# dpfried/action-segmentation

Measured on AMD Instinct MI355X. Metric: frames/sec semi-Markov decode, CrossTask T~10k K~20 L=1024, 1/2/4/8 GPUs, higher is better.
Workload: dtype f64

## Files before the change

action-segmentation_amd/_lib.py:

```python
import ctypes
import os

HERE = os.path.dirname(os.path.abspath(__file__))
LIB_PATH = os.environ.get("SMM_LIB_PATH") or os.path.join(HERE, "libsmmdp.so")

SYMBOLS = [
    "smm_strerror", "smm_last_hip_error", "smm_version", "smm_device_count", "smm_workspace_bytes",
    "smm_error_word_offset", "smm_dp_timing_enable", "smm_dp_timing_read", "smm_dp_timing_read_tagged", "smm_band_frame_ns", "smm_time_split_plan",
    "smm_env_reload", "smm_release_cached_plans", "smm_cached_plan_bytes", "smm_plan_feedback_info", "smm_plan_feedback_plan",
    "smm_emission_f64", "smm_emission_bwd_f64", "smm_viterbi_f64", "smm_viterbi_f32", "smm_decode_f32", "smm_logz_f64", "smm_logz_bwd_f64",
    "smm_sample_f64", "smm_entropy_f64", "smm_segment_posteriors_f64", "smm_kl_f64", "smm_kbest_workspace_bytes", "smm_kbest_f64",
    "smm_mbr_workspace_bytes", "smm_mbr_f64",
    "smm_align_workspace_bytes", "smm_align_f64", "smm_align_opt_workspace_bytes", "smm_align_opt_f64",
    "smm_align_graph_workspace_bytes", "smm_align_graph_f64",
    "smm_align_logz_workspace_bytes", "smm_align_logz_f64", "smm_align_logz_bwd_f64",
    "smm_align_opt_logz_workspace_bytes", "smm_align_opt_logz_f64", "smm_align_opt_logz_bwd_f64",
    "smm_align_graph_logz_workspace_bytes", "smm_align_graph_logz_f64", "smm_align_graph_logz_bwd_f64",
    "smm_align_graph_sample_f64", "smm_align_graph_entropy_f64", "smm_align_graph_kl_f64",
    "smm_align_graph_segment_posteriors_f64",
    "smm_entropy_bwd_scratch_bytes", "smm_entropy_bwd_f64", "smm_kl_bwd_f64",
    "smm_expected_reward_bwd_scratch_bytes", "smm_expected_reward_f64", "smm_expected_reward_bwd_f64",
    "smm_align_graph_entropy_bwd_scratch_bytes", "smm_align_graph_entropy_bwd_f64", "smm_align_graph_kl_bwd_f64",
    "smm_factor_tables_f64", "smm_factor_tables_bwd_f64",
    "smm_dense_workspace_bytes", "smm_dense_dp_f32", "smm_dense_marginals_f32",
    "smm_eval_workspace_bytes", "smm_eval_confusion_i64", "smm_eval_videos_i64",
    "smm_fit_workspace_bytes", "smm_fit_error_word_offset", "smm_fit_stats_f64",
]


class SmmShape(ctypes.Structure):
    _fields_ = [("b", ctypes.c_int32), ("d", ctypes.c_int32), ("n_groups", ctypes.c_int32),
                ("c_max", ctypes.c_int32), ("k_rows", ctypes.c_int32), ("t_max", ctypes.c_int32),
                ("flags", ctypes.c_int32), ("total_frames", ctypes.c_int64)]


class SmmPlanFeedbackInfo(ctypes.Structure):
    _fields_ = [("n_replans", ctypes.c_int32), ("n1_before", ctypes.c_int32), ("n1_after", ctypes.c_int32),
                ("n_videos", ctypes.c_int32), ("end_before_us", ctypes.c_double), ("end_after_us", ctypes.c_double),
                ("stamps", ctypes.POINTER(ctypes.c_uint64)), ("order", ctypes.POINTER(ctypes.c_int32))]


class SmmTablesShape(ctypes.Structure):
    _fields_ = [("n_classes", ctypes.c_int32), ("d", ctypes.c_int32), ("n_groups", ctypes.c_int32),
                ("c_max", ctypes.c_int32), ("k_rows", ctypes.c_int32), ("allow_self_transitions", ctypes.c_int32)]


SHAPE_NO_EOS = 1
SHAPE_LOGZ_BOTH = 2
SHAPE_NO_TIME_SPLIT = 4
KL_BWD_CROSS_ENTROPY = 0
KL_BWD_KL = 1
MAX_TRANSCRIPT = 256
ALIGN_LOGZ_TILE = 768

# ... 146 lines not shown
    lib.smm_band_frame_ns.restype = ctypes.c_double
    lib.smm_band_frame_ns.argtypes = [ctypes.c_int]
    lib.smm_time_split_plan.restype = ctypes.c_int
    lib.smm_time_split_plan.argtypes = [ctypes.POINTER(SmmShape)] + [ctypes.c_void_p] * 4 + [ctypes.c_int] + [ctypes.c_void_p] * 4 + [ctypes.c_int]
    lib.smm_env_reload.restype = None
    lib.smm_env_reload.argtypes = []
    lib.smm_release_cached_plans.restype = ctypes.c_size_t
    lib.smm_release_cached_plans.argtypes = []
    lib.smm_cached_plan_bytes.restype = ctypes.c_size_t
    lib.smm_cached_plan_bytes.argtypes = []
    lib.smm_plan_feedback_info.restype = ctypes.c_int
    lib.smm_plan_feedback_info.argtypes = [ctypes.POINTER(SmmPlanFeedbackInfo)]
    lib.smm_plan_feedback_plan.restype = ctypes.c_int
    lib.smm_plan_feedback_plan.argtypes = [ctypes.c_int, ctypes.c_int, ctypes.c_double] + [ctypes.c_void_p] * 3 + [ctypes.c_int, ctypes.c_int] \
        + [ctypes.c_void_p] * 4
    _lib = lib
    return lib


def reload_env():
    if _lib is not None:
        _lib.smm_env_reload()


def check(status):
    if status != 0:
        lib = load()
        msg = lib.smm_strerror(status).decode()
        if status == -4:
            msg += " (hipError %d)" % lib.smm_last_hip_error()
# ... 24 lines not shown
```

action-segmentation_amd/csrc/smm_api.hip:

```cpp
#include <algorithm>
#include <atomic>
#include <functional>
#include <cstdio>
#include <cstdlib>
#include <cstring>
#include <numeric>
#include <vector>
#include <unordered_map>
#include <mutex>
#include <utility>
#include <string>

#include "../../include/smmdp.h"
#include "smm_device.h"
#include "smm_launch.h"
#include "smm_plan_feedback.h"

static thread_local int g_last_hip = 0;

namespace {
struct SmmEnv {
    int spec = 1;
    int no_split = 0;
    double split_min_us = 100.0, split_ns = 0.0;
    int split_margin = 400;
    int plan_cache = 1;
    int small_wg = 1;
    int plan_feedback = 1;
    int chunk = 1;
    int chunk_p = 0;
    int chunk_lmin = 0;
    int chunk_wc = 512;
    int no_bt_window = 0;
    int fit_grid = 0;
    int verbose = 0;
#ifdef SMM_DEV
    int debug_flags = 0;
    int split_debug = 0;
    int upload_memcpy = 0;
    int emission_v2 = 0;
#endif
    std::string key;
};
std::atomic<const SmmEnv *> g_env{nullptr};
std::once_flag g_env_once;

void env_read()
{
    SmmEnv e;
    struct Item { const char *name; int *i; double *d; };
    const Item items[] = {
        {"SMM_SPEC", &e.spec, nullptr}, {"SMM_NO_SPLIT", &e.no_split, nullptr}, {"SMM_SPLIT_MIN_US", nullptr, &e.split_min_us},
        {"SMM_SPLIT_NS", nullptr, &e.split_ns}, {"SMM_SPLIT_MARGIN", &e.split_margin, nullptr},
        {"SMM_PLAN_CACHE", &e.plan_cache, nullptr}, {"SMM_SMALL_WG", &e.small_wg, nullptr}, {"SMM_PLAN_FEEDBACK", &e.plan_feedback, nullptr}, {"SMM_CHUNK", &e.chunk, nullptr}, {"SMM_CHUNK_P", &e.chunk_p, nullptr},
        {"SMM_CHUNK_WC", &e.chunk_wc, nullptr}, {"SMM_CHUNK_LMIN", &e.chunk_lmin, nullptr}, {"SMM_NO_BT_WINDOW", &e.no_bt_window, nullptr},
        {"SMM_FIT_GRID", &e.fit_grid, nullptr}, {"SMM_VERBOSE", &e.verbose, nullptr},
#ifdef SMM_DEV
        {"SMM_DEBUG_FLAGS", &e.debug_flags, nullptr}, {"SMM_SPLIT_DEBUG", &e.split_debug, nullptr},
        {"SMM_UPLOAD_MEMCPY", &e.upload_memcpy, nullptr}, {"SMM_EMISSION_V2", &e.emission_v2, nullptr},
#endif
    };
    for (const Item &it : items) {
        const char *v = std::getenv(it.name);
        if (!v) continue;
        if (it.i) *it.i = (*v == 0) ? 1 : std::atoi(v);
        if (it.d) *it.d = std::atof(v);
        e.key += it.name; e.key += '='; e.key += v; e.key += ';';
    }
// ... 238 lines not shown
struct Staged {
    SmmVideo *videos;
    int32_t *order;
    int32_t *n_states;
    int32_t *err;
    double *hist;
    double *elp;
    double *tabs;
    double *band;
    bool band_mode;
    int32_t *em_cum;
    std::vector<int32_t> em_cum_host;
    int em_tpw, em_blocks;
    int kp_max, c_need;
    int n_split;
    SmmVideo *uvideos;
    int32_t *uorder, *porder;
    SmmChunkVideo *cvs;
    int32_t *redo;
    double *anchors;
    int n_cv, n_units, u_part1;
    int small_first, small_count;
    uint64_t *stamps = nullptr;
    hipEvent_t done = nullptr;
    void *fb_entry = nullptr;
    std::vector<int32_t> order_host, frames_host;
};

static bool band_mode(int kp_max, int c_need);

// ... 22 lines not shown
    const SmmEnv &ev = env();
    if (b < 24 || ev.no_split) return 0;
    const int n_cu = device_cus();
    if (n_cu <= 0) return 0;
    const double em_us = (double)total_frames * (4.0 * d + 8.0 * c_max) / 4.0e6;
    if (em_us < ev.split_min_us) return 0;
    int tmax = 0;
    for (int i = 0; i < b; ++i) tmax = std::max(tmax, hv[i].T);
    const double split_ns = ev.split_ns > 0.0 ? ev.split_ns : 1.75 * smm_band_frame_ns(std::min(c_max, (int)SMM_MAX_STATES));
    const int thr = tmax - (int)(em_us * 1000.0 / split_ns) - ev.split_margin;
    int n1 = 0;
    for (int i = 0; i < b; ++i) n1 += hv[i].T >= thr;
    if (thr <= 0 || n1 < 1 || n1 > b / 3 || n1 > n_cu / 2 || b - n1 < 16 || b > 2 * n_cu) return 0;
    std::stable_partition(order, order + b, [&](int32_t v) { return hv[v].T >= thr; });
    return n1;
}

namespace {
struct PlanFeedback {
    uint64_t *stamps = nullptr;
    hipEvent_t done = nullptr;
    bool pending = false;
    bool have = false;
    bool busy = false;
    int evals_left = 5, n_replans = 0;
    int b = 0, n1_first = 0;
    double em_us = 0.0, end_before_us = 0.0, end_after_us = 0.0;
    std::vector<uint64_t> snap, used;
    std::vector<int32_t> order, frames;
};
// ... 273 lines not shown
{
    std::lock_guard<std::mutex> lock(g_plans.mu);
    size_t n = g_plans.pinned_bytes;
    for (int d = 0; d < 64; ++d)
        for (auto &ps : g_plans.slabs[d].all) n += ps.second;
    return n;
}

namespace {
struct FeedbackInfo {
    uint64_t generation = 0;
    smm_plan_feedback_info_t info{};
};
thread_local FeedbackInfo g_fb_info;

void feedback_info_set(const PlanFeedback *fb, int n1_now)
{
    g_fb_info.generation = g_plans.generation;
    smm_plan_feedback_info_t &o = g_fb_info.info;
    o.n_replans = fb->n_replans;
    o.n1_before = fb->n1_first;
    o.n1_after = n1_now;
    o.n_videos = fb->b;
    o.end_before_us = fb->end_before_us;
    o.end_after_us = fb->end_after_us;
    o.stamps = fb->used.empty() ? nullptr : fb->used.data();
    o.order = fb->order.data();
}

void feedback_evaluate(const Staged &st, hipStream_t stream)
{
    PlanEntry *e = static_cast<PlanEntry *>(st.fb_entry);
    if (!e || !e->fb) return;
    PlanFeedback *fb = e->fb;
    std::vector<uint64_t> snap;
    std::vector<int32_t> order;
    int n1 = 0;
    {
        std::lock_guard<std::mutex> lock(g_plans.mu);
        if (!fb->have || fb->busy || fb->evals_left <= 0) { feedback_info_set(fb, e->st.n_split); return; }
        fb->busy = true;
        snap = fb->snap;
        order = fb->order;
        n1 = e->st.n_split;
    }
    const SmmEnv &ev = env();
    const int b = fb->b, n_cu = device_cus();
    std::vector<double> dur(b);
    for (int i = 0; i < b; ++i) dur[i] = (double)(snap[2 * i + 1] - snap[2 * i]) * 0.01;
    const bool force = ev.plan_feedback >= 2;
    double em_us = fb->em_us;
    {
        uint64_t s1 = ~0ull, s2 = ~0ull;
        double f1 = 0.0, f_all = 0.0;
        for (int i = 0; i < b; ++i) {
            const int v = order[i];
            (i < n1 ? s1 : s2) = std::min(i < n1 ? s1 : s2, snap[2 * (size_t)v]);
            f_all += fb->frames[v];
            if (i < n1) f1 += fb->frames[v];
        }
        if (s2 > s1 && f_all > f1) em_us = std::min(2.0 * fb->em_us, std::max(0.5 * fb->em_us, (double)(s2 - s1) * 0.01 * f_all / (f_all - f1)));
    }
    const SmmFeedbackPlan plan = smm_feedback_plan(dur.data(), fb->frames.data(), order.data(), b, n1, n_cu, em_us, force);
    const bool planned = smm_feedback_guards(b, n_cu, plan.n1) && plan.end_chosen_us > 0.0;
    bool replan = planned && (force || (plan.changed && plan.end_chosen_us <= (1.0 - SMM_FEEDBACK_MIN_GAIN) * plan.end_current_us));
    const size_t o_cum = align_up(sizeof(int32_t) * (size_t)b, 256), bytes = o_cum + align_up(sizeof(int32_t) * ((size_t)b + 1), 256);
    std::vector<char> host(replan ? bytes : 0, 0);
    std::vector<int32_t> cum(replan ? b + 1 : 0);
    if (replan) {
        int64_t c = 0;
        for (int i = 0; i < b; ++i) { cum[i] = (int32_t)c; c += smm_emission_blocks(fb->frames[plan.order[i]], st.em_tpw); }
        cum[b] = (int32_t)c;
        if (c != st.em_blocks) replan = false;
        else {
            std::memcpy(host.data(), plan.order.data(), sizeof(int32_t) * b);
            std::memcpy(host.data() + o_cum, cum.data(), sizeof(int32_t) * ((size_t)b + 1));
        }
    }
    std::lock_guard<std::mutex> lock(g_plans.mu);
    fb->busy = false;
    fb->have = false;
    fb->evals_left -= 1;
    fb->used = std::move(snap);
    if (fb->n_replans == 0) fb->end_before_us = plan.end_current_us;
    fb->end_after_us = plan.end_current_us;
    char *dst = nullptr;
    if (replan && g_plans.bytes + bytes <= SMM_PLAN_MAX_BYTES) dst = plan_alloc(bytes, e->device);
    if (dst && smm_upload_meta(dst, host.data(), bytes, stream) == (int)hipSuccess && hipEventRecord(e->ready, stream) == hipSuccess) {
        g_plans.bytes += align_up(bytes, 256);
        e->st.order = reinterpret_cast<int32_t *>(dst);
        e->st.em_cum = reinterpret_cast<int32_t *>(dst + o_cum);
        e->st.em_cum_host = cum;
        e->st.n_split = plan.n1;
        e->stream = stream;
        e->settled = false;
        fb->order = plan.order;
        fb->n_replans += 1;
        fb->end_after_us = plan.end_chosen_us;
        if (force || fb->n_replans >= SMM_FEEDBACK_MAX_REPLANS) fb->evals_left = 0;
    } else {
        if (dst) (void)hipGetLastError();
        fb->evals_left = 0;
    }
    feedback_info_set(fb, e->st.n_split);
}
}

extern "C" int smm_plan_feedback_info(smm_plan_feedback_info_t *out)
{
    if (!out) return SMM_ERR_ARG;
    std::lock_guard<std::mutex> lock(g_plans.mu);
    *out = g_fb_info.generation == g_plans.generation ? g_fb_info.info : smm_plan_feedback_info_t{};
    return SMM_OK;
}

extern "C" int smm_plan_feedback_plan(int b, int n_cu, double em_us, const double *dur_us, const int32_t *frames,
                                      const int32_t *cur_order, int cur_n1, int force, int32_t *order_out, int32_t *n1_out,
                                      double *end_current_us, double *end_chosen_us)
{
    if (b < 1 || n_cu < 1 || !dur_us || !frames || !cur_order || cur_n1 < 0 || cur_n1 > b) return SMM_ERR_ARG;
    std::vector<char> seen(b, 0);
    for (int i = 0; i < b; ++i) {
        if (cur_order[i] < 0 || cur_order[i] >= b || seen[cur_order[i]]) return SMM_ERR_ARG;
        seen[cur_order[i]] = 1;
    }
    const SmmFeedbackPlan p = smm_feedback_plan(dur_us, frames, cur_order, b, cur_n1, n_cu, em_us, force != 0);
    if (order_out) std::memcpy(order_out, p.order.data(), sizeof(int32_t) * b);
    if (n1_out) *n1_out = p.n1;
    if (end_current_us) *end_current_us = p.end_current_us;
    if (end_chosen_us) *end_chosen_us = p.end_chosen_us;
    return p.changed ? 1 : 0;
}

struct ChunkPlan {
    std::vector<SmmVideo> units;
    std::vector<SmmChunkVideo> cvs;
};

static void plan_chunks_lmin(const smm_shape *s, const SmmVideo *hv, const int32_t *n_states, int kp_max, bool band, ChunkPlan &out, int n_cu_given, int lmin_cfg)
{
    const SmmEnv &ev = env();
    if (!ev.chunk || (s->flags & (SMM_SHAPE_NO_EOS | SMM_SHAPE_NO_TIME_SPLIT)) || kp_max <= 64) return;
    const int n_cu = n_cu_given > 0 ? n_cu_given : device_cus();
    if (n_cu <= 0) return;
    auto ns = [&](int c) { return dp_frame_ns(band, c); };
    double t_cu = 0.0, t_long = 0.0;
// ... 98 lines not shown
    }
    std::iota(ho, ho + s->b, 0);
    out->band_mode = band_mode(kp_max, c_need);
    const bool band = out->band_mode;
    std::stable_sort(ho, ho + s->b, [&](int a, int b) {
        return hv[a].T * dp_frame_ns(band, n_states[hv[a].group]) > hv[b].T * dp_frame_ns(band, n_states[hv[b].group]);
    });
    if (cum_chunk > 0) std::stable_sort(ho, ho + s->b, [&](int a, int b) { return hv[a].group < hv[b].group; });
    std::memcpy(hn, n_states, sizeof(int32_t) * s->n_groups);
    ChunkPlan cp;
    if (for_viterbi && cum_chunk == 0) plan_chunks(s, hv, n_states, kp_max, out->band_mode, cp);
    const int n_cv = (int)cp.cvs.size(), n_un = (int)cp.units.size();
    out->n_cv = n_cv;
    out->n_units = s->b - n_cv + n_un;
    out->u_part1 = n_un;
    out->n_split = 0;
    if (n_cv > 0) {
        std::vector<char> is_cv(s->b, 0);
        for (const SmmChunkVideo &cv : cp.cvs) is_cv[cv.vid] = 1;
        std::stable_partition(ho, ho + s->b, [&](int32_t v) { return is_cv[v] != 0; });
        const SmmEnv &ev = env();
        const double em_us = (double)s->total_frames * (4.0 * s->d + 8.0 * s->c_max) / 4.0e6;
        if (want_split && !ev.no_split && s->b - n_cv >= 16 && em_us >= ev.split_min_us) out->n_split = n_cv;
    } else {
        out->n_split = want_split ? choose_split(hv, ho, s->b, s->d, s->c_max, s->total_frames) : 0;
    }
    out->small_first = out->small_count = 0;
    if (for_viterbi && cum_chunk == 0 && out->band_mode && env().small_wg && !(s->flags & SMM_SHAPE_NO_EOS)) {
        const bool force = env().small_wg >= 2;
        const int n_cu = device_cus();
        const int t0 = out->n_split > 0 ? out->n_split : n_cv;
        const int n_tail = s->b - t0;
        if (n_cu > 0 && (force || n_tail >= 3 * n_cu)) {
            double t_cu = 0.0;
            for (int i = t0; i < s->b; ++i) t_cu += (double)hv[ho[i]].T * smm_band_frame_ns(n_states[hv[ho[i]].group]);
            t_cu /= n_cu;
            auto small = [&](int32_t v) {
                return n_states[hv[v].group] <= 16 && (force || (double)hv[v].T * 1.6 * smm_band_frame_ns(n_states[hv[v].group]) <= 0.5 * t_cu);
            };
            const int n_small = (int)std::count_if(ho + t0, ho + s->b, small);
// ... 401 lines not shown
    if (!elp || !trans || !init || !len_scores) return SMM_ERR_ARG;
    const size_t g = shape->n_groups, cm = shape->c_max;
    double *t64 = st.tabs, *i64 = t64 + g * cm * cm, *l64 = i64 + g * cm, *e64 = l64 + g * shape->k_rows * cm;
    smm_launch_widen(trans, t64, g * cm * cm, hs);
    smm_launch_widen(init, i64, g * cm, hs);
    smm_launch_widen(len_scores, l64, g * shape->k_rows * cm, hs);
    if (endpen) smm_launch_widen(endpen, e64, (size_t)shape->b * cm, hs);
    smm_launch_widen(elp, st.elp, (size_t)shape->total_frames * cm, hs);
    SMM_HIP(hipGetLastError());
    return run_viterbi(shape, st, st.elp, t64, i64, l64, endpen ? e64 : nullptr, class_map, spans, labels, best, n_segs, hs);
}

namespace {
struct AuxDev {
    hipStream_t stream = nullptr, stream1 = nullptr;
    std::vector<std::pair<hipEvent_t, hipEvent_t>> events;
};
std::mutex g_aux_mu;
AuxDev g_aux[64];

hipStream_t aux_stream_n(int dev, int which)
{
    std::lock_guard<std::mutex> lock(g_aux_mu);
    AuxDev &d = g_aux[dev];
    hipStream_t &st = which ? d.stream1 : d.stream;
    if (!st) {
        int least = 0, greatest = 0;
        (void)hipDeviceGetStreamPriorityRange(&least, &greatest);
        if (hipStreamCreateWithPriority(&st, hipStreamNonBlocking, least) != hipSuccess) st = nullptr;
    }
    return st;
}
hipStream_t aux_stream(int dev) { return aux_stream_n(dev, 0); }

bool aux_events_get(int dev, std::pair<hipEvent_t, hipEvent_t> &ev)
{
    {
        std::lock_guard<std::mutex> lock(g_aux_mu);
        AuxDev &d = g_aux[dev];
        if (!d.events.empty()) { ev = d.events.back(); d.events.pop_back(); return true; }
    }
    ev = {nullptr, nullptr};
    if (hipEventCreateWithFlags(&ev.first, hipEventDisableTiming) != hipSuccess) return false;
    if (hipEventCreateWithFlags(&ev.second, hipEventDisableTiming) != hipSuccess) { (void)hipEventDestroy(ev.first); return false; }
// ... 3 lines not shown
void aux_events_put(int dev, const std::pair<hipEvent_t, hipEvent_t> &ev)
{
    std::lock_guard<std::mutex> lock(g_aux_mu);
    g_aux[dev].events.push_back(ev);
}
}

static void release_aux()
{
    std::lock_guard<std::mutex> lock(g_aux_mu);
    for (int d = 0; d < 64; ++d) {
        for (auto &ev : g_aux[d].events) { (void)hipEventDestroy(ev.first); (void)hipEventDestroy(ev.second); }
        g_aux[d].events.clear();
        if (g_aux[d].stream) { (void)hipStreamDestroy(g_aux[d].stream); g_aux[d].stream = nullptr; }
        if (g_aux[d].stream1) { (void)hipStreamDestroy(g_aux[d].stream1); g_aux[d].stream1 = nullptr; }
    }
    std::lock_guard<std::mutex> lock2(g_dp_timing.mu);
    for (auto &ev : g_dp_timing.pool) { (void)hipEventDestroy(ev.first); (void)hipEventDestroy(ev.second); }
    g_dp_timing.pool.clear();
}

extern "C" int smm_decode_f32(const smm_shape *shape, const int64_t *lengths_host, const int64_t *frame_offset_host,
                              const int32_t *group_host, const int32_t *kp_host, const int32_t *n_states_host,
                              const float *x, const double *w, const double *cst, const double *inv_var, const float *cons,
                              const double *trans, const double *init, const double *len_scores, const double *endpen,
                              const int64_t *class_map, int64_t *spans, int64_t *labels, double *best, int32_t *n_segs,
                              float *elp32, void *workspace, size_t workspace_bytes, void *stream)
{
    g_fb_info = FeedbackInfo{};
    Staged st;
// ... 5 lines not shown
    hipStream_t aux = nullptr;
    if (st.n_split > 0 && hipGetDevice(&dev) == hipSuccess && dev >= 0 && dev < 64) {
        hipStreamCaptureStatus cap = hipStreamCaptureStatusNone;
        if (hipStreamIsCapturing(hs, &cap) == hipSuccess && cap == hipStreamCaptureStatusNone) aux = aux_stream(dev);
    }
    std::pair<hipEvent_t, hipEvent_t> fj{nullptr, nullptr};
    if (aux && !aux_events_get(dev, fj)) aux = nullptr;
    if (!aux) {
        rc = run_emission(shape, st, x, w, cst, inv_var, cons, st.elp, elp32, hs);
        if (rc != SMM_OK) return rc;
        rc = run_viterbi(shape, st, st.elp, trans, init, len_scores, endpen, class_map, spans, labels, best, n_segs, hs);
        if (st.stamps && hipEventRecord(st.done, hs) != hipSuccess) (void)hipGetLastError();
        return rc;
    }
    const int n1 = st.n_split, n2 = shape->b - st.n_split;
    rc = run_viterbi(shape, st, st.elp, trans, init, len_scores, endpen, class_map, spans, labels, best, n_segs, hs, 0, n1, true, false);
    if (rc != SMM_OK) { aux_events_put(dev, fj); return rc; }
    const hipEvent_t fork = fj.first, join = fj.second;
    int rc2 = SMM_OK;
    rc = run_emission(shape, st, x, w, cst, inv_var, cons, st.elp, elp32, hs, 0, n1);
    if (rc != SMM_OK) { aux_events_put(dev, fj); return rc; }
    if (hipEventRecord(fork, hs) != hipSuccess || hipStreamWaitEvent(aux, fork, 0) != hipSuccess) rc2 = SMM_ERR_HIP;
#ifdef SMM_DEV
    const int dbg_split = env().split_debug;
#else
    const int dbg_split = 0;
#endif
    if (rc2 == SMM_OK && !(dbg_split & 2)) rc2 = run_emission(shape, st, x, w, cst, inv_var, cons, st.elp, elp32, aux, n1, n2);
    if (rc2 == SMM_OK && !(dbg_split & 1))
        rc2 = run_viterbi(shape, st, st.elp, trans, init, len_scores, endpen, class_map, spans, labels, best, n_segs, aux, n1, n2, false, true, 2);
    rc = run_viterbi(shape, st, st.elp, trans, init, len_scores, endpen, class_map, spans, labels, best, n_segs, hs, 0, n1, false, true, 1);
    if (hipEventRecord(join, aux) != hipSuccess || hipStreamWaitEvent(hs, join, 0) != hipSuccess) rc2 = SMM_ERR_HIP;
    aux_events_put(dev, fj);
    if (st.stamps && hipEventRecord(st.done, hs) != hipSuccess) (void)hipGetLastError();
    if (rc == SMM_OK && rc2 == SMM_OK) feedback_evaluate(st, hs);
    return rc != SMM_OK ? rc : rc2;
}

extern "C" int smm_logz_f64(const smm_shape *shape, const int64_t *lengths_host, const int64_t *frame_offset_host,
                            const int32_t *group_host, const int32_t *kp_host, const int32_t *n_states_host,
                            const double *elp, const double *trans, const double *init, const double *len_scores,
                            const double *endpen, double *logz, void *workspace, size_t workspace_bytes, void *stream)
{
    Staged st;
    hipStream_t hs = static_cast<hipStream_t>(stream);
    int rc = stage(shape, lengths_host, frame_offset_host, group_host, kp_host, n_states_host, workspace, workspace_bytes,
                   hs, &st);
    if (rc != SMM_OK) return rc;
// ... 1151 lines not shown
```

action-segmentation_amd/csrc/smm_plan_feedback.h:

```cpp
#pragma once
#include <algorithm>
#include <cstdint>
#include <functional>
#include <numeric>
#include <queue>
#include <vector>

struct SmmFeedbackPlan {
    int n1 = 0;
    std::vector<int32_t> order;
    double end_current_us = 0.0;
    double end_chosen_us = 0.0;
    bool changed = false;
};

inline bool smm_feedback_guards(int b, int n_cu, int n1)
{
    return b >= 24 && n_cu > 0 && n1 >= 1 && n1 <= b / 3 && n1 <= n_cu / 2 && b - n1 >= 16;
}

inline double smm_feedback_replay(const double *dur_us, const int32_t *frames, const int32_t *order, int b, int n1, int n_cu,
                                  double em_us)
{
    if (b < 1 || n1 < 1 || n1 >= b || n1 >= n_cu) return 0.0;
    double f1 = 0.0, f_all = 0.0;
    for (int i = 0; i < b; ++i) {
        f_all += (double)frames[order[i]];
        if (i < n1) f1 += (double)frames[order[i]];
    }
    const double em1 = f_all > 0.0 ? em_us * f1 / f_all : 0.0;
    double end = 0.0;
    std::vector<double> free_at;
    free_at.reserve(n_cu);
    for (int i = 0; i < n1; ++i) {
        const double e = em1 + dur_us[order[i]];
        end = std::max(end, e);
        free_at.push_back(std::max(e, em_us));
    }
    const int direct = std::min(b, n_cu);
    for (int i = n1; i < direct; ++i) {
        const double e = em_us + dur_us[order[i]];
        end = std::max(end, e);
        free_at.push_back(e);
    }
    if (direct < b) {
        std::priority_queue<double, std::vector<double>, std::greater<double>> cus(std::greater<double>(), std::move(free_at));
        for (int i = direct; i < b; ++i) {
            const double e = cus.top() + dur_us[order[i]];
            cus.pop();
            cus.push(e);
            end = std::max(end, e);
        }
    }
    return end;
}

inline SmmFeedbackPlan smm_feedback_plan(const double *dur_us, const int32_t *frames, const int32_t *cur_order, int b, int cur_n1,
                                         int n_cu, double em_us, bool force = false)
{
    SmmFeedbackPlan out;
    out.n1 = cur_n1;
    out.order.assign(cur_order, cur_order + b);
    out.end_current_us = out.end_chosen_us = smm_feedback_replay(dur_us, frames, cur_order, b, cur_n1, n_cu, em_us);
    if (!smm_feedback_guards(b, n_cu, cur_n1)) return out;
    std::vector<int32_t> by_time(cur_order, cur_order + b);
    std::stable_sort(by_time.begin(), by_time.end(), [&](int32_t x, int32_t y) { return dur_us[x] > dur_us[y]; });
    int best_n1 = 0;
    double best_end = 0.0;
    for (int step = 0; step <= b; ++step) {
        const int n1 = step == 0 ? cur_n1 : step;
        if ((step > 0 && n1 == cur_n1) || !smm_feedback_guards(b, n_cu, n1)) continue;
        const double e = smm_feedback_replay(dur_us, frames, by_time.data(), b, n1, n_cu, em_us);
        if (best_n1 == 0 || e < best_end) { best_n1 = n1; best_end = e; }
    }
    if (best_n1 == 0) return out;
    if (!force && !(best_end < out.end_current_us)) return out;
    out.n1 = best_n1;
    out.end_chosen_us = best_end;
    out.changed = best_n1 != cur_n1 || !std::equal(by_time.begin(), by_time.end(), cur_order);
    out.order = std::move(by_time);
    return out;
}
```

action-segmentation_amd/ops.py:

```python
import ctypes

import numpy as np
import torch

from . import _lib
from ._lib import SmmShape


class Batch:

    def __init__(self, lengths, n_states, k_rows, c_max=None, frame_offset=None, group=None, kp=None, d=0,
                 t_max=None, total_frames=None, no_eos=False, no_time_split=False):
        self.lengths = np.ascontiguousarray(np.asarray(lengths, dtype=np.int64).reshape(-1))
        self.b = int(self.lengths.shape[0])
        self.n_states = np.ascontiguousarray(np.asarray(n_states, dtype=np.int32).reshape(-1))
        self.n_groups = int(self.n_states.shape[0])
        self.c_max = int(c_max if c_max is not None else self.n_states.max())
        self.k_rows = int(k_rows)
        self.t_max = int(t_max if t_max is not None else self.lengths.max())
        if frame_offset is None:
            frame_offset = np.arange(self.b, dtype=np.int64) * self.t_max
        self.frame_offset = np.ascontiguousarray(np.asarray(frame_offset, dtype=np.int64).reshape(-1))
        self.group = None if group is None else np.ascontiguousarray(np.asarray(group, dtype=np.int32).reshape(-1))
        self.kp = None if kp is None else np.ascontiguousarray(np.asarray(kp, dtype=np.int32).reshape(-1))
# ... 1314 lines not shown
    buf = (ctypes.c_float * cap)()
    tags = (ctypes.c_int32 * cap)()
    n = _lib.load().smm_dp_timing_read_tagged(buf, tags, cap)
    if tagged:
        return [(float(buf[i]), int(tags[i])) for i in range(min(n, cap))]
    return [float(buf[i]) for i in range(min(n, cap))]


def plan_feedback_info():
    import numpy as np
    info = _lib.SmmPlanFeedbackInfo()
    _lib.check(_lib.load().smm_plan_feedback_info(ctypes.byref(info)))
    n = int(info.n_videos)
    stamps = np.ctypeslib.as_array(info.stamps, shape=(n, 2)).astype(np.int64) if n > 0 and info.stamps else None
    order = np.ctypeslib.as_array(info.order, shape=(n,)).copy() if n > 0 and info.order else None
    return {'n_replans': int(info.n_replans), 'n1_before': int(info.n1_before), 'n1_after': int(info.n1_after), 'n_videos': n,
            'end_before_us': float(info.end_before_us), 'end_after_us': float(info.end_after_us), 'stamps': stamps, 'order': order}


def plan_feedback_plan(dur_us, frames, cur_order, cur_n1, n_cu, em_us, force=False):
    import numpy as np
    dur = np.ascontiguousarray(dur_us, dtype=np.float64)
    fr = np.ascontiguousarray(frames, dtype=np.int32)
    cur = np.ascontiguousarray(cur_order, dtype=np.int32)
    b = len(dur)
    if len(fr) != b or len(cur) != b:
        raise ValueError("dur_us, frames and cur_order must have one entry per video")
    order = np.zeros(b, dtype=np.int32)
    n1 = ctypes.c_int32(0)
    e0, e1 = ctypes.c_double(0.0), ctypes.c_double(0.0)
    ptr = lambda a: ctypes.c_void_p(a.ctypes.data)
    rc = _lib.load().smm_plan_feedback_plan(b, int(n_cu), float(em_us), ptr(dur), ptr(fr), ptr(cur), int(cur_n1), 1 if force else 0,
                                            ptr(order), ctypes.cast(ctypes.byref(n1), ctypes.c_void_p),
                                            ctypes.cast(ctypes.byref(e0), ctypes.c_void_p), ctypes.cast(ctypes.byref(e1), ctypes.c_void_p))
    if rc < 0:
        _lib.check(rc)
    return bool(rc), order, int(n1.value), float(e0.value), float(e1.value)


def time_split_plan(batch, n_cu=256):
    import numpy as np
    lib = _lib.load()
    ln, fo, gr, kp, ns = batch.host_ptrs()
    cap = int(batch.total_frames // 128 + 2 * batch.b + 8)
    arrs = [np.zeros(cap, dtype=np.int32) for _ in range(4)]
    n = lib.smm_time_split_plan(ctypes.byref(batch.shape), ctypes.c_void_p(ln), ctypes.c_void_p(gr), ctypes.c_void_p(kp), ctypes.c_void_p(ns),
                                int(n_cu), *[ctypes.c_void_p(a.ctypes.data) for a in arrs], cap)
    if n < 0:
        raise _lib.SmmError("smm_time_split_plan: %s" % lib.smm_strerror(n).decode())
    return [tuple(int(a[i]) for a in arrs) for i in range(min(n, cap))]


def reload_env():
    _lib.reload_env()
# ... 10 lines not shown
```

include/smmdp.h:

```cpp
#ifndef SMMDP_H
#define SMMDP_H

#include <stddef.h>
#include <stdint.h>

#ifdef __cplusplus
extern "C" {
#endif

typedef enum smm_status {
    SMM_OK = 0,
    SMM_ERR_ARG = -1,
    SMM_ERR_UNSUPPORTED = -2,
    SMM_ERR_WORKSPACE = -3,
    SMM_ERR_HIP = -4,
    SMM_ERR_NO_DEVICE = -5
} smm_status;

#define SMM_MAX_STATES 32
#define SMM_MAX_K_ROWS 1024

typedef struct smm_shape {
    int32_t b;
    int32_t d;
// ... 29 lines not shown

double smm_band_frame_ns(int n_states);

size_t smm_release_cached_plans(void);
size_t smm_cached_plan_bytes(void);
void smm_env_reload(void);

typedef struct smm_plan_feedback_info_t {
    int32_t n_replans;
    int32_t n1_before, n1_after;
    int32_t n_videos;
    double end_before_us;
    double end_after_us;
    const uint64_t *stamps;
    const int32_t *order;
} smm_plan_feedback_info_t;
int smm_plan_feedback_info(smm_plan_feedback_info_t *out);

int smm_plan_feedback_plan(int b, int n_cu, double em_us, const double *dur_us, const int32_t *frames, const int32_t *cur_order,
                           int cur_n1, int force, int32_t *order_out, int32_t *n1_out, double *end_current_us,
                           double *end_chosen_us);

int smm_emission_f64(const smm_shape *shape, const int64_t *lengths_host, const int64_t *frame_offset_host,
                     const int32_t *group_host, const int32_t *n_states_host,
                     const float *x, const double *w, const double *cst, const double *inv_var, const float *cons,
                     double *elp64, float *elp32, void *workspace, size_t workspace_bytes, void *stream);

int smm_emission_bwd_f64(const smm_shape *shape, const int64_t *lengths_host, const int64_t *frame_offset_host,
                         const int32_t *group_host, const int32_t *n_states_host,
                         const float *x, const double *g_elp, double *g_w, double *g_cst, double *g_inv_var,
                         void *workspace, size_t workspace_bytes, void *stream);

int smm_viterbi_f64(const smm_shape *shape, const int64_t *lengths_host, const int64_t *frame_offset_host,
                    const int32_t *group_host, const int32_t *kp_host, const int32_t *n_states_host,
                    const double *elp, const double *trans, const double *init, const double *len_scores,
                    const double *endpen, const int64_t *class_map,
// ... 320 lines not shown
```

Measured before the change: 1.002 billion.

## Start Viterbi of longest head videos on high-priority stream before remaining emission

Adds a 'head' subset of the longest videos within the first split part. Emission runs for those first, then their Viterbi launches on a new high-priority stream while emission for the rest of part one and the second part continue. The goal is to shorten the critical path set by the single longest video. The feedback planner gains a head-aware replay model to choose n1 and n0 together. The cost is an extra stream and events, more launches, and planner complexity.

```diff
diff --git a/action-segmentation_amd/_lib.py b/action-segmentation_amd/_lib.py
--- a/action-segmentation_amd/_lib.py
+++ b/action-segmentation_amd/_lib.py
@@ -7,7 +7,7 @@
 SYMBOLS = [
     "smm_strerror", "smm_last_hip_error", "smm_version", "smm_device_count", "smm_workspace_bytes",
     "smm_error_word_offset", "smm_dp_timing_enable", "smm_dp_timing_read", "smm_dp_timing_read_tagged", "smm_band_frame_ns", "smm_time_split_plan",
-    "smm_env_reload", "smm_release_cached_plans", "smm_cached_plan_bytes", "smm_plan_feedback_info", "smm_plan_feedback_plan",
+    "smm_env_reload", "smm_release_cached_plans", "smm_cached_plan_bytes", "smm_plan_feedback_info", "smm_plan_feedback_plan", "smm_plan_feedback_plan_head", "smm_plan_feedback_replay_head",
     "smm_emission_f64", "smm_emission_bwd_f64", "smm_viterbi_f64", "smm_viterbi_f32", "smm_decode_f32", "smm_logz_f64", "smm_logz_bwd_f64",
     "smm_sample_f64", "smm_entropy_f64", "smm_segment_posteriors_f64", "smm_kl_f64", "smm_kbest_workspace_bytes", "smm_kbest_f64",
     "smm_mbr_workspace_bytes", "smm_mbr_f64",
@@ -37,7 +37,8 @@
 class SmmPlanFeedbackInfo(ctypes.Structure):
     _fields_ = [("n_replans", ctypes.c_int32), ("n1_before", ctypes.c_int32), ("n1_after", ctypes.c_int32),
                 ("n_videos", ctypes.c_int32), ("end_before_us", ctypes.c_double), ("end_after_us", ctypes.c_double),
-                ("stamps", ctypes.POINTER(ctypes.c_uint64)), ("order", ctypes.POINTER(ctypes.c_int32))]
+                ("stamps", ctypes.POINTER(ctypes.c_uint64)), ("order", ctypes.POINTER(ctypes.c_int32)),
+                ("n0_after", ctypes.c_int32)]
 
 
 class SmmTablesShape(ctypes.Structure):
@@ -214,6 +215,11 @@
     lib.smm_plan_feedback_plan.restype = ctypes.c_int
     lib.smm_plan_feedback_plan.argtypes = [ctypes.c_int, ctypes.c_int, ctypes.c_double] + [ctypes.c_void_p] * 3 + [ctypes.c_int, ctypes.c_int] \
         + [ctypes.c_void_p] * 4
+    lib.smm_plan_feedback_plan_head.restype = ctypes.c_int
+    lib.smm_plan_feedback_plan_head.argtypes = [ctypes.c_int, ctypes.c_int, ctypes.c_double, ctypes.c_double] + [ctypes.c_void_p] * 3 \
+        + [ctypes.c_int] * 3 + [ctypes.c_void_p] * 5
+    lib.smm_plan_feedback_replay_head.restype = ctypes.c_double
+    lib.smm_plan_feedback_replay_head.argtypes = [ctypes.c_int, ctypes.c_int, ctypes.c_double] + [ctypes.c_void_p] * 3 + [ctypes.c_int] * 2
     _lib = lib
     return lib
 
diff --git a/action-segmentation_amd/csrc/smm_api.hip b/action-segmentation_amd/csrc/smm_api.hip
--- a/action-segmentation_amd/csrc/smm_api.hip
+++ b/action-segmentation_amd/csrc/smm_api.hip
@@ -24,6 +24,8 @@
     int no_split = 0;
     double split_min_us = 100.0, split_ns = 0.0;
     int split_margin = 400;
+    int head = 1;
+    double head_min_us = 40.0;
     int plan_cache = 1;
     int small_wg = 1;
     int plan_feedback = 1;
@@ -52,6 +54,7 @@
     const Item items[] = {
         {"SMM_SPEC", &e.spec, nullptr}, {"SMM_NO_SPLIT", &e.no_split, nullptr}, {"SMM_SPLIT_MIN_US", nullptr, &e.split_min_us},
         {"SMM_SPLIT_NS", nullptr, &e.split_ns}, {"SMM_SPLIT_MARGIN", &e.split_margin, nullptr},
+        {"SMM_HEAD", &e.head, nullptr}, {"SMM_HEAD_MIN_US", nullptr, &e.head_min_us},
         {"SMM_PLAN_CACHE", &e.plan_cache, nullptr}, {"SMM_SMALL_WG", &e.small_wg, nullptr}, {"SMM_PLAN_FEEDBACK", &e.plan_feedback, nullptr}, {"SMM_CHUNK", &e.chunk, nullptr}, {"SMM_CHUNK_P", &e.chunk_p, nullptr},
         {"SMM_CHUNK_WC", &e.chunk_wc, nullptr}, {"SMM_CHUNK_LMIN", &e.chunk_lmin, nullptr}, {"SMM_NO_BT_WINDOW", &e.no_bt_window, nullptr},
         {"SMM_FIT_GRID", &e.fit_grid, nullptr}, {"SMM_VERBOSE", &e.verbose, nullptr},
@@ -320,6 +323,7 @@
     int em_tpw, em_blocks;
     int kp_max, c_need;
     int n_split;
+    int n_head = 0;
     SmmVideo *uvideos;
     int32_t *uorder, *porder;
     SmmChunkVideo *cvs;
@@ -372,6 +376,21 @@
     if (thr <= 0 || n1 < 1 || n1 > b / 3 || n1 > n_cu / 2 || b - n1 < 16 || b > 2 * n_cu) return 0;
     std::stable_partition(order, order + b, [&](int32_t v) { return hv[v].T >= thr; });
     return n1;
+}
+
+static int choose_head(const SmmVideo *hv, const int32_t *order, const int32_t *n_states, int b, int n1, bool band, int d, int c_max,
+                       int64_t total_frames)
+{
+    const SmmEnv &ev = env();
+    if (!ev.head || n1 < 2) return 0;
+    std::vector<double> dur(b);
+    std::vector<int32_t> frames(b);
+    for (int i = 0; i < b; ++i) {
+        frames[i] = hv[i].T;
+        dur[i] = (double)hv[i].T * dp_frame_ns(band, n_states[hv[i].group]) * 1e-3;
+    }
+    const double em_us = (double)total_frames * (4.0 * d + 8.0 * c_max) / 4.0e6;
+    return smm_feedback_head_size(dur.data(), frames.data(), order, b, n1, em_us, ev.head_min_us);
 }
 
 namespace {
@@ -675,13 +694,14 @@
 };
 thread_local FeedbackInfo g_fb_info;
 
-void feedback_info_set(const PlanFeedback *fb, int n1_now)
+void feedback_info_set(const PlanFeedback *fb, int n1_now, int n0_now)
 {
     g_fb_info.generation = g_plans.generation;
     smm_plan_feedback_info_t &o = g_fb_info.info;
     o.n_replans = fb->n_replans;
     o.n1_before = fb->n1_first;
     o.n1_after = n1_now;
+    o.n0_after = n0_now;
     o.n_videos = fb->b;
     o.end_before_us = fb->end_before_us;
     o.end_after_us = fb->end_after_us;
@@ -689,6 +709,8 @@
     o.order = fb->order.data();
 }
 
+hipStream_t aux_stream_n(int dev, int which);
+
 void feedback_evaluate(const Staged &st, hipStream_t stream)
 {
     PlanEntry *e = static_cast<PlanEntry *>(st.fb_entry);
@@ -696,16 +718,19 @@
     PlanFeedback *fb = e->fb;
     std::vector<uint64_t> snap;
     std::vector<int32_t> order;
-    int n1 = 0;
+    int n1 = 0, n0 = 0;
     {
         std::lock_guard<std::mutex> lock(g_plans.mu);
-        if (!fb->have || fb->busy || fb->evals_left <= 0) { feedback_info_set(fb, e->st.n_split); return; }
+        if (!fb->have || fb->busy || fb->evals_left <= 0) { feedback_info_set(fb, e->st.n_split, e->st.n_head); return; }
         fb->busy = true;
         snap = fb->snap;
         order = fb->order;
         n1 = e->st.n_split;
+        n0 = e->st.n_head;
     }
     const SmmEnv &ev = env();
+    const bool with_head = ev.head && e->device >= 0 && e->device < 64 && aux_stream_n(e->device, 2) != nullptr;
+    if (!with_head) n0 = 0;
     const int b = fb->b, n_cu = device_cus();
     std::vector<double> dur(b);
     for (int i = 0; i < b; ++i) dur[i] = (double)(snap[2 * i + 1] - snap[2 * i]) * 0.01;
@@ -716,13 +741,16 @@
         double f1 = 0.0, f_all = 0.0;
         for (int i = 0; i < b; ++i) {
             const int v = order[i];
-            (i < n1 ? s1 : s2) = std::min(i < n1 ? s1 : s2, snap[2 * (size_t)v]);
+            if (i >= n0) (i < n1 ? s1 : s2) = std::min(i < n1 ? s1 : s2, snap[2 * (size_t)v]);
             f_all += fb->frames[v];
             if (i < n1) f1 += fb->frames[v];
         }
         if (s2 > s1 && f_all > f1) em_us = std::min(2.0 * fb->em_us, std::max(0.5 * fb->em_us, (double)(s2 - s1) * 0.01 * f_all / (f_all - f1)));
     }
-    const SmmFeedbackPlan plan = smm_feedback_plan(dur.data(), fb->frames.data(), order.data(), b, n1, n_cu, em_us, force);
+    SmmFeedbackHeadPlan hp;
+    if (with_head) hp = smm_feedback_plan_head(dur.data(), fb->frames.data(), order.data(), b, n1, n0, n_cu, em_us, ev.head_min_us, force);
+    else hp.plan = smm_feedback_plan(dur.data(), fb->frames.data(), order.data(), b, n1, n_cu, em_us, force);
+    const SmmFeedbackPlan &plan = hp.plan;
     const bool planned = smm_feedback_guards(b, n_cu, plan.n1) && plan.end_chosen_us > 0.0;
     bool replan = planned && (force || (plan.changed && plan.end_chosen_us <= (1.0 - SMM_FEEDBACK_MIN_GAIN) * plan.end_current_us));
     const size_t o_cum = align_up(sizeof(int32_t) * (size_t)b, 256), bytes = o_cum + align_up(sizeof(int32_t) * ((size_t)b + 1), 256);
@@ -753,6 +781,7 @@
         e->st.em_cum = reinterpret_cast<int32_t *>(dst + o_cum);
         e->st.em_cum_host = cum;
         e->st.n_split = plan.n1;
+        e->st.n_head = hp.n0;
         e->stream = stream;
         e->settled = false;
         fb->order = plan.order;
@@ -763,7 +792,7 @@
         if (dst) (void)hipGetLastError();
         fb->evals_left = 0;
     }
-    feedback_info_set(fb, e->st.n_split);
+    feedback_info_set(fb, e->st.n_split, e->st.n_head);
 }
 }
 
@@ -791,6 +820,33 @@
     if (end_current_us) *end_current_us = p.end_current_us;
     if (end_chosen_us) *end_chosen_us = p.end_chosen_us;
     return p.changed ? 1 : 0;
+}
+
+extern "C" int smm_plan_feedback_plan_head(int b, int n_cu, double em_us, double min_tail_us, const double *dur_us, const int32_t *frames,
+                                           const int32_t *cur_order, int cur_n1, int cur_n0, int force, int32_t *order_out,
+                                           int32_t *n1_out, int32_t *n0_out, double *end_current_us, double *end_chosen_us)
+{
+    if (b < 1 || n_cu < 1 || !dur_us || !frames || !cur_order || cur_n1 < 0 || cur_n1 > b || cur_n0 < 0 || cur_n0 > cur_n1) return SMM_ERR_ARG;
+    std::vector<char> seen(b, 0);
+    for (int i = 0; i < b; ++i) {
+        if (cur_order[i] < 0 || cur_order[i] >= b || seen[cur_order[i]]) return SMM_ERR_ARG;
+        seen[cur_order[i]] = 1;
+    }
+    const SmmFeedbackHeadPlan p = smm_feedback_plan_head(dur_us, frames, cur_order, b, cur_n1, cur_n0, n_cu, em_us, min_tail_us, force != 0);
+    if (order_out) std::memcpy(order_out, p.plan.order.data(), sizeof(int32_t) * b);
+    if (n1_out) *n1_out = p.plan.n1;
+    if (n0_out) *n0_out = p.n0;
+    if (end_current_us) *end_current_us = p.plan.end_current_us;
+    if (end_chosen_us) *end_chosen_us = p.plan.end_chosen_us;
+    return p.plan.changed ? 1 : 0;
+}
+
+extern "C" double smm_plan_feedback_replay_head(int b, int n_cu, double em_us, const double *dur_us, const int32_t *frames,
+                                                const int32_t *order, int n1, int n0)
+{
+    if (b < 1 || n_cu < 1 || !dur_us || !frames || !order) return 0.0;
+    for (int i = 0; i < b; ++i) if (order[i] < 0 || order[i] >= b) return 0.0;
+    return smm_feedback_replay_head(dur_us, frames, order, b, n1, n0, n_cu, em_us);
 }
 
 struct ChunkPlan {
@@ -919,7 +975,7 @@
     out->n_cv = n_cv;
     out->n_units = s->b - n_cv + n_un;
     out->u_part1 = n_un;
-    out->n_split = 0;
+    out->n_split = out->n_head = 0;
     if (n_cv > 0) {
         std::vector<char> is_cv(s->b, 0);
         for (const SmmChunkVideo &cv : cp.cvs) is_cv[cv.vid] = 1;
@@ -929,6 +985,7 @@
         if (want_split && !ev.no_split && s->b - n_cv >= 16 && em_us >= ev.split_min_us) out->n_split = n_cv;
     } else {
         out->n_split = want_split ? choose_split(hv, ho, s->b, s->d, s->c_max, s->total_frames) : 0;
+        if (out->n_split > 0) out->n_head = choose_head(hv, ho, n_states, s->b, out->n_split, band, s->d, s->c_max, s->total_frames);
     }
     out->small_first = out->small_count = 0;
     if (for_viterbi && cum_chunk == 0 && out->band_mode && env().small_wg && !(s->flags & SMM_SHAPE_NO_EOS)) {
@@ -1360,6 +1417,8 @@
 namespace {
 struct AuxDev {
     hipStream_t stream = nullptr, stream1 = nullptr;
+    hipStream_t stream2 = nullptr;
+    bool no_stream2 = false;
     std::vector<std::pair<hipEvent_t, hipEvent_t>> events;
 };
 std::mutex g_aux_mu;
@@ -1369,11 +1428,16 @@
 {
     std::lock_guard<std::mutex> lock(g_aux_mu);
     AuxDev &d = g_aux[dev];
-    hipStream_t &st = which ? d.stream1 : d.stream;
-    if (!st) {
+    hipStream_t &st = which == 2 ? d.stream2 : which ? d.stream1 : d.stream;
+    if (!st && !(which == 2 && d.no_stream2)) {
         int least = 0, greatest = 0;
-        (void)hipDeviceGetStreamPriorityRange(&least, &greatest);
-        if (hipStreamCreateWithPriority(&st, hipStreamNonBlocking, least) != hipSuccess) st = nullptr;
+        const bool ranged = hipDeviceGetStreamPriorityRange(&least, &greatest) == hipSuccess;
+        if (which == 2 && !(ranged && least - greatest >= 2)) d.no_stream2 = true;
+        else if (hipStreamCreateWithPriority(&st, hipStreamNonBlocking, which == 2 ? greatest : least) != hipSuccess) {
+            (void)hipGetLastError();
+            st = nullptr;
+            if (which == 2) d.no_stream2 = true;
+        }
     }
     return st;
 }
@@ -1407,6 +1471,8 @@
         g_aux[d].events.clear();
         if (g_aux[d].stream) { (void)hipStreamDestroy(g_aux[d].stream); g_aux[d].stream = nullptr; }
         if (g_aux[d].stream1) { (void)hipStreamDestroy(g_aux[d].stream1); g_aux[d].stream1 = nullptr; }
+        if (g_aux[d].stream2) { (void)hipStreamDestroy(g_aux[d].stream2); g_aux[d].stream2 = nullptr; }
+        g_aux[d].no_stream2 = false;
     }
     std::lock_guard<std::mutex> lock2(g_dp_timing.mu);
     for (auto &ev : g_dp_timing.pool) { (void)hipEventDestroy(ev.first); (void)hipEventDestroy(ev.second); }
@@ -1442,24 +1508,40 @@
         return rc;
     }
     const int n1 = st.n_split, n2 = shape->b - st.n_split;
+    hipStream_t head = nullptr;
+    std::pair<hipEvent_t, hipEvent_t> hj{nullptr, nullptr};
+    if (st.n_head > 0 && st.n_head < n1 && st.n_cv == 0) head = aux_stream_n(dev, 2);
+    if (head && !aux_events_get(dev, hj)) head = nullptr;
+    const int n0 = head ? st.n_head : 0;
+    if (env().verbose) std::fprintf(stderr, "smm_decode_f32: %d videos, first part %d, head %d (planned %d)\n", shape->b, n1, n0, st.n_head);
+    auto put_events = [&]() { aux_events_put(dev, fj); if (head) aux_events_put(dev, hj); };
     rc = run_viterbi(shape, st, st.elp, trans, init, len_scores, endpen, class_map, spans, labels, best, n_segs, hs, 0, n1, true, false);
-    if (rc != SMM_OK) { aux_events_put(dev, fj); return rc; }
+    if (rc != SMM_OK) { put_events(); return rc; }
     const hipEvent_t fork = fj.first, join = fj.second;
-    int rc2 = SMM_OK;
-    rc = run_emission(shape, st, x, w, cst, inv_var, cons, st.elp, elp32, hs, 0, n1);
-    if (rc != SMM_OK) { aux_events_put(dev, fj); return rc; }
-    if (hipEventRecord(fork, hs) != hipSuccess || hipStreamWaitEvent(aux, fork, 0) != hipSuccess) rc2 = SMM_ERR_HIP;
+    int rc2 = SMM_OK, rc0 = SMM_OK;
+    rc = run_emission(shape, st, x, w, cst, inv_var, cons, st.elp, elp32, hs, 0, n0 > 0 ? n0 : n1);
+    if (rc != SMM_OK) { put_events(); return rc; }
+    if (n0 > 0) {
+        if (hipEventRecord(hj.first, hs) != hipSuccess || hipStreamWaitEvent(head, hj.first, 0) != hipSuccess) rc0 = SMM_ERR_HIP;
+        else rc0 = run_viterbi(shape, st, st.elp, trans, init, len_scores, endpen, class_map, spans, labels, best, n_segs, head, 0, n0, false, true, 1);
+        rc = run_emission(shape, st, x, w, cst, inv_var, cons, st.elp, elp32, hs, n0, n1 - n0);
+    }
+    if (rc == SMM_OK) {
+        if (hipEventRecord(fork, hs) != hipSuccess || hipStreamWaitEvent(aux, fork, 0) != hipSuccess) rc2 = SMM_ERR_HIP;
 #ifdef SMM_DEV
-    const int dbg_split = env().split_debug;
+        const int dbg_split = env().split_debug;
 #else
-    const int dbg_split = 0;
+        const int dbg_split = 0;
 #endif
-    if (rc2 == SMM_OK && !(dbg_split & 2)) rc2 = run_emission(shape, st, x, w, cst, inv_var, cons, st.elp, elp32, aux, n1, n2);
-    if (rc2 == SMM_OK && !(dbg_split & 1))
-        rc2 = run_viterbi(shape, st, st.elp, trans, init, len_scores, endpen, class_map, spans, labels, best, n_segs, aux, n1, n2, false, true, 2);
-    rc = run_viterbi(shape, st, st.elp, trans, init, len_scores, endpen, class_map, spans, labels, best, n_segs, hs, 0, n1, false, true, 1);
-    if (hipEventRecord(join, aux) != hipSuccess || hipStreamWaitEvent(hs, join, 0) != hipSuccess) rc2 = SMM_ERR_HIP;
-    aux_events_put(dev, fj);
+        if (rc2 == SMM_OK && !(dbg_split & 2)) rc2 = run_emission(shape, st, x, w, cst, inv_var, cons, st.elp, elp32, aux, n1, n2);
+        if (rc2 == SMM_OK && !(dbg_split & 1))
+            rc2 = run_viterbi(shape, st, st.elp, trans, init, len_scores, endpen, class_map, spans, labels, best, n_segs, aux, n1, n2, false, true, 2);
+        rc = run_viterbi(shape, st, st.elp, trans, init, len_scores, endpen, class_map, spans, labels, best, n_segs, hs, n0, n1 - n0, false, true, 1);
+        if (hipEventRecord(join, aux) != hipSuccess || hipStreamWaitEvent(hs, join, 0) != hipSuccess) rc2 = SMM_ERR_HIP;
+    }
+    if (n0 > 0 && (hipEventRecord(hj.second, head) != hipSuccess || hipStreamWaitEvent(hs, hj.second, 0) != hipSuccess)) rc0 = SMM_ERR_HIP;
+    put_events();
+    if (rc == SMM_OK) rc = rc0;
     if (st.stamps && hipEventRecord(st.done, hs) != hipSuccess) (void)hipGetLastError();
     if (rc == SMM_OK && rc2 == SMM_OK) feedback_evaluate(st, hs);
     return rc != SMM_OK ? rc : rc2;
diff --git a/action-segmentation_amd/csrc/smm_plan_feedback.h b/action-segmentation_amd/csrc/smm_plan_feedback.h
--- a/action-segmentation_amd/csrc/smm_plan_feedback.h
+++ b/action-segmentation_amd/csrc/smm_plan_feedback.h
@@ -19,21 +19,23 @@
     return b >= 24 && n_cu > 0 && n1 >= 1 && n1 <= b / 3 && n1 <= n_cu / 2 && b - n1 >= 16;
 }
 
-inline double smm_feedback_replay(const double *dur_us, const int32_t *frames, const int32_t *order, int b, int n1, int n_cu,
-                                  double em_us)
+inline double smm_feedback_replay_head(const double *dur_us, const int32_t *frames, const int32_t *order, int b, int n1, int n0,
+                                       int n_cu, double em_us)
 {
-    if (b < 1 || n1 < 1 || n1 >= b || n1 >= n_cu) return 0.0;
-    double f1 = 0.0, f_all = 0.0;
+    if (b < 1 || n1 < 1 || n1 >= b || n1 >= n_cu || n0 < 0 || n0 >= n1) return 0.0;
+    double f0 = 0.0, f1 = 0.0, f_all = 0.0;
     for (int i = 0; i < b; ++i) {
         f_all += (double)frames[order[i]];
         if (i < n1) f1 += (double)frames[order[i]];
+        if (i < n0) f0 += (double)frames[order[i]];
     }
     const double em1 = f_all > 0.0 ? em_us * f1 / f_all : 0.0;
+    const double em_head = f_all > 0.0 ? em_us * f0 / f_all : 0.0;
     double end = 0.0;
     std::vector<double> free_at;
     free_at.reserve(n_cu);
     for (int i = 0; i < n1; ++i) {
-        const double e = em1 + dur_us[order[i]];
+        const double e = (i < n0 ? em_head : em1) + dur_us[order[i]];
         end = std::max(end, e);
         free_at.push_back(std::max(e, em_us));
     }
@@ -53,6 +55,12 @@
         }
     }
     return end;
+}
+
+inline double smm_feedback_replay(const double *dur_us, const int32_t *frames, const int32_t *order, int b, int n1, int n_cu,
+                                  double em_us)
+{
+    return smm_feedback_replay_head(dur_us, frames, order, b, n1, 0, n_cu, em_us);
 }
 
 inline SmmFeedbackPlan smm_feedback_plan(const double *dur_us, const int32_t *frames, const int32_t *cur_order, int b, int cur_n1,
@@ -81,3 +89,57 @@
     out.order = std::move(by_time);
     return out;
 }
+
+inline int smm_feedback_head_size(const double *dur_us, const int32_t *frames, const int32_t *order, int b, int n1, double em_us,
+                                  double min_tail_us)
+{
+    if (b < 1 || n1 < 2 || n1 > b) return 0;
+    double f_all = 0.0, f_tail = 0.0;
+    for (int i = 0; i < b; ++i) f_all += (double)frames[order[i]];
+    for (int i = 1; i < n1; ++i) f_tail += (double)frames[order[i]];
+    if (!(f_all > 0.0)) return 0;
+    const double t0 = dur_us[order[0]], margin = 0.015 * t0;
+    for (int n = 1; n < n1; ++n) {
+        const double em_tail = em_us * f_tail / f_all;
+        if (dur_us[order[n]] <= t0 - em_tail - margin) return em_tail >= min_tail_us ? n : 0;
+        f_tail -= (double)frames[order[n]];
+    }
+    return 0;
+}
+
+struct SmmFeedbackHeadPlan {
+    SmmFeedbackPlan plan;
+    int n0 = 0;
+};
+
+inline SmmFeedbackHeadPlan smm_feedback_plan_head(const double *dur_us, const int32_t *frames, const int32_t *cur_order, int b,
+                                                  int cur_n1, int cur_n0, int n_cu, double em_us, double min_tail_us,
+                                                  bool force = false)
+{
+    SmmFeedbackHeadPlan out;
+    SmmFeedbackPlan &p = out.plan;
+    out.n0 = cur_n0;
+    p.n1 = cur_n1;
+    p.order.assign(cur_order, cur_order + b);
+    p.end_current_us = p.end_chosen_us = smm_feedback_replay_head(dur_us, frames, cur_order, b, cur_n1, cur_n0, n_cu, em_us);
+    if (!smm_feedback_guards(b, n_cu, cur_n1)) return out;
+    std::vector<int32_t> by_time(cur_order, cur_order + b);
+    std::stable_sort(by_time.begin(), by_time.end(), [&](int32_t x, int32_t y) { return dur_us[x] > dur_us[y]; });
+    int best_n1 = 0, best_n0 = 0;
+    double best_end = 0.0;
+    for (int step = 0; step <= b; ++step) {
+        const int n1 = step == 0 ? cur_n1 : step;
+        if ((step > 0 && n1 == cur_n1) || !smm_feedback_guards(b, n_cu, n1)) continue;
+        const int n0 = smm_feedback_head_size(dur_us, frames, by_time.data(), b, n1, em_us, min_tail_us);
+        const double e = smm_feedback_replay_head(dur_us, frames, by_time.data(), b, n1, n0, n_cu, em_us);
+        if (best_n1 == 0 || e < best_end) { best_n1 = n1; best_n0 = n0; best_end = e; }
+    }
+    if (best_n1 == 0) return out;
+    if (!force && !(best_end < p.end_current_us)) return out;
+    p.n1 = best_n1;
+    out.n0 = best_n0;
+    p.end_chosen_us = best_end;
+    p.changed = best_n1 != cur_n1 || best_n0 != cur_n0 || !std::equal(by_time.begin(), by_time.end(), cur_order);
+    p.order = std::move(by_time);
+    return out;
+}
diff --git a/action-segmentation_amd/ops.py b/action-segmentation_amd/ops.py
--- a/action-segmentation_amd/ops.py
+++ b/action-segmentation_amd/ops.py
@@ -1352,7 +1352,8 @@
     n = int(info.n_videos)
     stamps = np.ctypeslib.as_array(info.stamps, shape=(n, 2)).astype(np.int64) if n > 0 and info.stamps else None
     order = np.ctypeslib.as_array(info.order, shape=(n,)).copy() if n > 0 and info.order else None
-    return {'n_replans': int(info.n_replans), 'n1_before': int(info.n1_before), 'n1_after': int(info.n1_after), 'n_videos': n,
+    return {'n_replans': int(info.n_replans), 'n1_before': int(info.n1_before), 'n1_after': int(info.n1_after), 'n0_after': int(info.n0_after),
+            'n_videos': n,
             'end_before_us': float(info.end_before_us), 'end_after_us': float(info.end_after_us), 'stamps': stamps, 'order': order}
 
 
@@ -1376,6 +1377,37 @@
     return bool(rc), order, int(n1.value), float(e0.value), float(e1.value)
 
 
+def plan_feedback_plan_head(dur_us, frames, cur_order, cur_n1, cur_n0, n_cu, em_us, min_tail_us=40.0, force=False):
+    import numpy as np
+    dur = np.ascontiguousarray(dur_us, dtype=np.float64)
+    fr = np.ascontiguousarray(frames, dtype=np.int32)
+    cur = np.ascontiguousarray(cur_order, dtype=np.int32)
+    b = len(dur)
+    if len(fr) != b or len(cur) != b:
+        raise ValueError("dur_us, frames and cur_order must have one entry per video")
+    order = np.zeros(b, dtype=np.int32)
+    n1, n0 = ctypes.c_int32(0), ctypes.c_int32(0)
+    e0, e1 = ctypes.c_double(0.0), ctypes.c_double(0.0)
+    ptr = lambda a: ctypes.c_void_p(a.ctypes.data)
+    ref = lambda v: ctypes.cast(ctypes.byref(v), ctypes.c_void_p)
+    rc = _lib.load().smm_plan_feedback_plan_head(b, int(n_cu), float(em_us), float(min_tail_us), ptr(dur), ptr(fr), ptr(cur), int(cur_n1),
+                                                 int(cur_n0), 1 if force else 0, ptr(order), ref(n1), ref(n0), ref(e0), ref(e1))
+    if rc < 0:
+        _lib.check(rc)
+    return bool(rc), order, int(n1.value), int(n0.value), float(e0.value), float(e1.value)
+
+
+def plan_feedback_replay_head(dur_us, frames, order, n1, n0, n_cu, em_us):
+    import numpy as np
+    dur = np.ascontiguousarray(dur_us, dtype=np.float64)
+    fr = np.ascontiguousarray(frames, dtype=np.int32)
+    od = np.ascontiguousarray(order, dtype=np.int32)
+    if len(fr) != len(dur) or len(od) != len(dur):
+        raise ValueError("dur_us, frames and order must have one entry per video")
+    ptr = lambda a: ctypes.c_void_p(a.ctypes.data)
+    return float(_lib.load().smm_plan_feedback_replay_head(len(dur), int(n_cu), float(em_us), ptr(dur), ptr(fr), ptr(od), int(n1), int(n0)))
+
+
 def time_split_plan(batch, n_cu=256):
     import numpy as np
     lib = _lib.load()
diff --git a/include/smmdp.h b/include/smmdp.h
--- a/include/smmdp.h
+++ b/include/smmdp.h
@@ -67,12 +67,19 @@
     double end_after_us;
     const uint64_t *stamps;
     const int32_t *order;
+    int32_t n0_after;
 } smm_plan_feedback_info_t;
 int smm_plan_feedback_info(smm_plan_feedback_info_t *out);
 
 int smm_plan_feedback_plan(int b, int n_cu, double em_us, const double *dur_us, const int32_t *frames, const int32_t *cur_order,
                            int cur_n1, int force, int32_t *order_out, int32_t *n1_out, double *end_current_us,
                            double *end_chosen_us);
+
+int smm_plan_feedback_plan_head(int b, int n_cu, double em_us, double min_tail_us, const double *dur_us, const int32_t *frames,
+                                const int32_t *cur_order, int cur_n1, int cur_n0, int force, int32_t *order_out, int32_t *n1_out,
+                                int32_t *n0_out, double *end_current_us, double *end_chosen_us);
+double smm_plan_feedback_replay_head(int b, int n_cu, double em_us, const double *dur_us, const int32_t *frames,
+                                     const int32_t *order, int n1, int n0);
 
 int smm_emission_f64(const smm_shape *shape, const int64_t *lengths_host, const int64_t *frame_offset_host,
                      const int32_t *group_host, const int32_t *n_states_host,
```

New measurement: 915.0 million. 8.7% lower.
